# vllm-project/production-stack

Hardware: AMD Instinct MI355X
Metric: output_tokens_per_sec (higher is better)
Workload: dtype bfloat16; 1 GPU; multi-round-qa; model=llama-3-8b, users_per_gpu=320, rounds_per_conversation=10, max_model_len=8192, parallelism=dp1, prefix_caching=True, kv_cache_dtype=auto, quantization=none

## Files before the change

### csrc/attention.hip

```cpp
#include "ps_common.h"

template <int HEAD_DIM, int GQ, int BLOCK_SIZE, int NWAVES, int LOWREG,
          typename KVT, int PIPE = 0>
__global__ __launch_bounds__(NWAVES * 64, LOWREG ? 3 : 1) void paged_attn_decode_kernel(
    unsigned short* __restrict__ out,
    float* __restrict__ ws_acc,
    float* __restrict__ ws_ml,
    const unsigned short* __restrict__ q,
    const KVT* __restrict__ k_cache,
    const KVT* __restrict__ v_cache,
    const int* __restrict__ block_tables,
    const int* __restrict__ seq_lens,
    const int* __restrict__ order,
    int max_blocks, float scale, int KH, long q_stride, int window) {
  using KVTr = ps_kv_traits<KVT>;
  using kvec8 = typename KVTr::vec8;
  constexpr int D = HEAD_DIM;
  constexpr int LPG = D / 8;
  constexpr int TPW = 64 / LPG;
  static_assert(BLOCK_SIZE % TPW == 0, "block size must divide");
  static_assert(!PIPE || LOWREG, "the pipelined loop is a LOWREG variant");

  const int seq = order ? order[blockIdx.x] : blockIdx.x;
  if ((unsigned)seq >= gridDim.x) return;
  const int kvh = blockIdx.y;
  const int ctx = seq_lens[seq];
  const int wave = threadIdx.x >> 6;
  const int lane = threadIdx.x & 63;
  const int sg = lane / LPG;
  const int sl = lane % LPG;

  ps_bf16x8 qp[GQ];
  const unsigned short* qbase = q + (long)seq * q_stride + (long)kvh * GQ * D;
#pragma unroll
  for (int g = 0; g < GQ; g++)
    qp[g] = *(const ps_bf16x8*)(qbase + g * D + sl * 8);
  float qf[GQ][8];
  if constexpr (!LOWREG) {
#pragma unroll
    for (int g = 0; g < GQ; g++)
#pragma unroll
      for (int j = 0; j < 8; j++) qf[g][j] = ps_bf16_to_f32(qp[g][j]);
  }

  float m[GQ], l[GQ], acc[GQ][8];
#pragma unroll
  for (int g = 0; g < GQ; g++) {
    m[g] = PS_NEG_INF;
    l[g] = 0.f;
#pragma unroll
    for (int j = 0; j < 8; j++) acc[g][j] = 0.f;
  }

  const int nblocks = (ctx + BLOCK_SIZE - 1) / BLOCK_SIZE;
  const int win_lo = (window > 0 && ctx > window) ? ctx - window : 0;
  const int first_block = win_lo / BLOCK_SIZE;
  const int nsplit = gridDim.z;
  const int split = blockIdx.z;
  const int live_blocks = nblocks - first_block;
  const int per_split = (live_blocks + nsplit - 1) / nsplit;
  const int b_begin = first_block + split * per_split;
  const int b_end = min(nblocks, b_begin + per_split);
  const int* bt = block_tables + (long)seq * max_blocks;
  constexpr int TPB = BLOCK_SIZE / TPW;
  if constexpr (PIPE != 0) {
    int b = b_begin + wave;
    if (b < b_end) {
      const int lane_off = sg * D + sl * 8;
      long blk = __builtin_amdgcn_readfirstlane(bt[b]);
      for (; b < b_end; b += NWAVES) {
        const long blk_next = __builtin_amdgcn_readfirstlane(
            bt[b + NWAVES < b_end ? b + NWAVES : b]);
        const KVT* kb = k_cache + ((blk * KH + kvh) * BLOCK_SIZE) * D;
        const KVT* vb = v_cache + ((blk * KH + kvh) * BLOCK_SIZE) * D;
        const int valid_tokens = min(BLOCK_SIZE, ctx - b * BLOCK_SIZE);
        float sc[GQ][TPB];
        kvec8 vv[TPB];
#pragma unroll
        for (int g = 0; g < GQ; g++)
          asm volatile("" : "+v"(qp[g]));
#pragma unroll
        for (int tt = 0; tt < TPB; tt++) {
          const int tok = tt * TPW + sg;
          const bool valid =
              tok < valid_tokens && b * BLOCK_SIZE + tok >= win_lo;
          kvec8 kv = *(const kvec8*)(kb + tt * TPW * D + lane_off);
          float kf[8];
          KVTr::to_f32x8(kv, kf);
#pragma unroll
          for (int g = 0; g < GQ; g++) {
            float s = 0.f;
#pragma unroll
            for (int j = 0; j < 8; j++)
              s += ps_bf16_to_f32(qp[g][j]) * kf[j];
            s = ps_group_sum<LPG>(s) * scale;
            sc[g][tt] = valid ? s : PS_NEG_INF;
          }
        }
#pragma unroll
        for (int tt = 0; tt < TPB; tt++)
          vv[tt] = *(const kvec8*)(vb + tt * TPW * D + lane_off);
#pragma unroll
        for (int g = 0; g < GQ; g++) {
          float bmax = sc[g][0];
#pragma unroll
          for (int tt = 1; tt < TPB; tt++) bmax = fmaxf(bmax, sc[g][tt]);
          const float mnew = fmaxf(m[g], bmax);
          const float corr = __expf(m[g] - mnew);
          float p[TPB];
          float psum = 0.f;
#pragma unroll
          for (int tt = 0; tt < TPB; tt++) {
            p[tt] = sc[g][tt] > PS_NEG_INF ? __expf(sc[g][tt] - mnew) : 0.f;
            psum += p[tt];
          }
          l[g] = l[g] * corr + psum;
#pragma unroll
          for (int j = 0; j < 8; j++) acc[g][j] *= corr;
#pragma unroll
          for (int tt = 0; tt < TPB; tt++) {
            float vf[8];
            KVTr::to_f32x8(vv[tt], vf);
#pragma unroll
            for (int j = 0; j < 8; j++) acc[g][j] += p[tt] * vf[j];
          }
          m[g] = mnew;
        }
        blk = blk_next;
      }
    }
  }
  for (int b = PIPE ? b_end : b_begin + wave; b < b_end; b += NWAVES) {
    const long blk = bt[b];
    const KVT* kb = k_cache + ((blk * KH + kvh) * BLOCK_SIZE) * D;
    const KVT* vb = v_cache + ((blk * KH + kvh) * BLOCK_SIZE) * D;
    const int valid_tokens = min(BLOCK_SIZE, ctx - b * BLOCK_SIZE);
    float sc[GQ][TPB];
    kvec8 vv[TPB];
    if constexpr (LOWREG) {
#pragma unroll
      for (int g = 0; g < GQ; g++)
        asm volatile("" : "+v"(qp[g]));
    }
#pragma unroll
    for (int tt = 0; tt < TPB; tt++) {
      const int tok = tt * TPW + sg;
      const bool valid =
          tok < valid_tokens && b * BLOCK_SIZE + tok >= win_lo;
      kvec8 kv = *(const kvec8*)(kb + tok * D + sl * 8);
      if constexpr (!LOWREG)
        vv[tt] = *(const kvec8*)(vb + tok * D + sl * 8);
      float kf[8];
      KVTr::to_f32x8(kv, kf);
#pragma unroll
      for (int g = 0; g < GQ; g++) {
        float s = 0.f;
#pragma unroll
        for (int j = 0; j < 8; j++) {
          if constexpr (LOWREG)
            s += ps_bf16_to_f32(qp[g][j]) * kf[j];
          else
            s += qf[g][j] * kf[j];
        }
        s = ps_group_sum<LPG>(s) * scale;
        sc[g][tt] = valid ? s : PS_NEG_INF;
      }
    }
    if constexpr (LOWREG) {
#pragma unroll
      for (int tt = 0; tt < TPB; tt++)
        vv[tt] = *(const kvec8*)(vb + (tt * TPW + sg) * D + sl * 8);
    }
#pragma unroll
    for (int g = 0; g < GQ; g++) {
      float bmax = sc[g][0];
#pragma unroll
      for (int tt = 1; tt < TPB; tt++) bmax = fmaxf(bmax, sc[g][tt]);
      const float mnew = fmaxf(m[g], bmax);
      const float corr = __expf(m[g] - mnew);
      float p[TPB];
      float psum = 0.f;
#pragma unroll
      for (int tt = 0; tt < TPB; tt++) {
        p[tt] = sc[g][tt] > PS_NEG_INF ? __expf(sc[g][tt] - mnew) : 0.f;
        psum += p[tt];
      }
      l[g] = l[g] * corr + psum;
#pragma unroll
      for (int j = 0; j < 8; j++) acc[g][j] *= corr;
#pragma unroll
      for (int tt = 0; tt < TPB; tt++) {
        float vf[8];
        KVTr::to_f32x8(vv[tt], vf);
#pragma unroll
        for (int j = 0; j < 8; j++) acc[g][j] += p[tt] * vf[j];
      }
      m[g] = mnew;
    }
  }

#pragma unroll
  for (int off = LPG; off < 64; off <<= 1) {
#pragma unroll
    for (int g = 0; g < GQ; g++) {
      const float mo = __shfl_xor(m[g], off, 64);
      const float lo = __shfl_xor(l[g], off, 64);
      const float mnew = fmaxf(m[g], mo);
      const float c1 = __expf(m[g] - mnew);
      const float c2 = __expf(mo - mnew);
#pragma unroll
      for (int j = 0; j < 8; j++) {
        const float ao = __shfl_xor(acc[g][j], off, 64);
        acc[g][j] = acc[g][j] * c1 + ao * c2;
      }
      l[g] = l[g] * c1 + lo * c2;
      m[g] = mnew;
    }
  }

  __shared__ float sm[NWAVES][GQ];
  __shared__ float slse[NWAVES][GQ];
  __shared__ float sacc[NWAVES][GQ][D];
  if (sg == 0) {
#pragma unroll
    for (int g = 0; g < GQ; g++) {
      if (sl == 0) {
        sm[wave][g] = m[g];
        slse[wave][g] = l[g];
      }
#pragma unroll
      for (int j = 0; j < 8; j++) sacc[wave][g][sl * 8 + j] = acc[g][j];
    }
  }
  __syncthreads();
  if (wave == 0 && sg == 0) {
#pragma unroll
    for (int g = 0; g < GQ; g++) {
      float M = PS_NEG_INF, L = 0.f, A[8];
#pragma unroll
      for (int j = 0; j < 8; j++) A[j] = 0.f;
#pragma unroll
      for (int wv = 0; wv < NWAVES; wv++) {
        const float mw = sm[wv][g];
        const float mnew = fmaxf(M, mw);
        const float c1 = __expf(M - mnew);
        const float c2 = __expf(mw - mnew);
        L = L * c1 + slse[wv][g] * c2;
#pragma unroll
        for (int j = 0; j < 8; j++)
          A[j] = A[j] * c1 + sacc[wv][g][sl * 8 + j] * c2;
        M = mnew;
      }
      const long head = (long)seq * KH * GQ + (long)kvh * GQ + g;
      if (nsplit == 1) {
        const float inv = L > 0.f ? 1.f / L : 0.f;
        ps_bf16x8 ov;
#pragma unroll
        for (int j = 0; j < 8; j++) ov[j] = ps_f32_to_bf16(A[j] * inv);
        *(ps_bf16x8*)(out + head * D + sl * 8) = ov;
      } else {
        float* wa = ws_acc + (head * nsplit + split) * D + sl * 8;
#pragma unroll
        for (int j = 0; j < 8; j++) wa[j] = A[j];
        if (sl == 0) {
          float* wm = ws_ml + (head * nsplit + split) * 2;
          wm[0] = M;
          wm[1] = L;
        }
      }
    }
  }
}

#define PS_DECODE_ORDER_MAX 4096
__global__ __launch_bounds__(1024) void decode_order_kernel(
    int* __restrict__ order,
    const int* __restrict__ seq_lens,
    int S) {
  __shared__ int lens[PS_DECODE_ORDER_MAX];
  for (int i = threadIdx.x; i < S; i += blockDim.x) lens[i] = seq_lens[i];
  __syncthreads();
// ... 86 lines not shown
    const long blk = bt[b];
    const unsigned short* kb = k_cache + ((blk * KH + kvh) * BLOCK_SIZE) * D;
    const unsigned short* vb = v_cache + ((blk * KH + kvh) * BLOCK_SIZE) * D;
    const int valid_tokens = min(BLOCK_SIZE, ctx - b * BLOCK_SIZE);
#pragma unroll
    for (int tt = 0; tt < BLOCK_SIZE / TPW; tt++) {
      const int tok = tt * TPW + sg;
      const bool valid =
          tok < valid_tokens && b * BLOCK_SIZE + tok >= win_lo;
      ps_bf16x8 kv = *(const ps_bf16x8*)(kb + tok * D + sl * 8);
      ps_bf16x8 vv = *(const ps_bf16x8*)(vb + tok * D + sl * 8);
      float s = 0.f;
#pragma unroll
      for (int j = 0; j < 8; j++) s += qf[j] * ps_bf16_to_f32(kv[j]);
      s = ps_group_sum<LPG>(s);
      const float sv = valid ? s : PS_NEG_INF;
      const float mnew = fmaxf(m, sv);
      const float corr = __expf(m - mnew);
      const float p = valid ? __expf(sv - mnew) : 0.f;
      l = l * corr + p;
#pragma unroll
      for (int j = 0; j < 8; j++)
        acc[j] = acc[j] * corr + p * ps_bf16_to_f32(vv[j]);
      m = mnew;
    }
  }

#pragma unroll
  for (int off = LPG; off < 64; off <<= 1) {
    const float mo = __shfl_xor(m, off, 64);
    const float lo = __shfl_xor(l, off, 64);
    const float mnew = fmaxf(m, mo);
    const float c1 = __expf(m - mnew);
    const float c2 = __expf(mo - mnew);
#pragma unroll
    for (int j = 0; j < 8; j++) {
      const float ao = __shfl_xor(acc[j], off, 64);
      acc[j] = acc[j] * c1 + ao * c2;
    }
    l = l * c1 + lo * c2;
    m = mnew;
  }
  if (sg == 0) {
    const float inv = l > 0.f ? 1.f / l : 0.f;
    ps_bf16x8 ov;
#pragma unroll
    for (int j = 0; j < 8; j++) ov[j] = ps_f32_to_bf16(acc[j] * inv);
    *(ps_bf16x8*)(out + ((long)tokid * QH + qh) * D + sl * 8) = ov;
  }
}

template <typename KVT>
__global__ void reshape_and_cache_kernel(
    const unsigned short* __restrict__ k,
    const unsigned short* __restrict__ v,
    KVT* __restrict__ k_cache,
    KVT* __restrict__ v_cache,
    const long* __restrict__ slot_mapping,
    int KH, int HD, int BS, long total ) {
  using KVTr = ps_kv_traits<KVT>;
  using kvec8 = typename KVTr::vec8;
  const long stride = (long)gridDim.x * blockDim.x;
  const int row = KH * HD;
  for (long idx = (long)blockIdx.x * blockDim.x + threadIdx.x; idx < total;
       idx += stride) {
    const long elem = idx * 8;
    const long t = elem / row;
    const int r = (int)(elem % row);
    const int h = r / HD;
    const int d = r % HD;
    const long slot = slot_mapping[t];
    if (slot < 0) continue;
    const long blk = slot / BS;
    const int off = (int)(slot % BS);
    const long dst = ((blk * KH + h) * BS + off) * (long)HD + d;
    ps_bf16x8 kv = *(const ps_bf16x8*)(k + elem);
    ps_bf16x8 vv = *(const ps_bf16x8*)(v + elem);
    kvec8 ko, vo;
#pragma unroll
    for (int j = 0; j < 8; j++) {
      ko[j] = KVTr::from_f32(ps_bf16_to_f32(kv[j]));
      vo[j] = KVTr::from_f32(ps_bf16_to_f32(vv[j]));
    }
    *(kvec8*)(k_cache + dst) = ko;
    *(kvec8*)(v_cache + dst) = vo;
  }
}

__global__ void greedy_sample_kernel(long* __restrict__ out,
                                     const unsigned short* __restrict__ logits,
                                     int V) {
  const long r = blockIdx.x;
  const unsigned short* row = logits + r * (long)V;
  float best = PS_NEG_INF;
  int besti = 0;
  for (int i = threadIdx.x * 8; i + 8 <= V; i += blockDim.x * 8) {
    ps_bf16x8 xv = *(const ps_bf16x8*)(row + i);
#pragma unroll
    for (int j = 0; j < 8; j++) {
      const float f = ps_bf16_to_f32(xv[j]);
      if (f > best) {
        best = f;
        besti = i + j;
      }
    }
  }
  const int tail_start = (V / 8) * 8;
  for (int i = tail_start + threadIdx.x; i < V; i += blockDim.x) {
    const float f = ps_bf16_to_f32(row[i]);
    if (f > best) {
      best = f;
      besti = i;
    }
  }
#pragma unroll
  for (int off = 32; off > 0; off >>= 1) {
    const float ob = __shfl_xor(best, off, 64);
    const int oi = __shfl_xor(besti, off, 64);
    if (ob > best || (ob == best && oi < besti)) {
      best = ob;
      besti = oi;
    }
  }
  __shared__ float wbest[4];
  __shared__ int wbesti[4];
  const int wave = threadIdx.x >> 6;
  if ((threadIdx.x & 63) == 0) {
    wbest[wave] = best;
    wbesti[wave] = besti;
  }
  __syncthreads();
  if (threadIdx.x == 0) {
    for (int wv = 1; wv < (int)(blockDim.x >> 6); wv++) {
      if (wbest[wv] > wbest[0] ||
          (wbest[wv] == wbest[0] && wbesti[wv] < wbesti[0])) {
        wbest[0] = wbest[wv];
        wbesti[0] = wbesti[wv];
      }
    }
    out[r] = wbesti[0];
  }
}

extern "C" {

int ps_paged_attn_decode(void* out, void* ws_acc, void* ws_ml, const void* q,
                         const void* k_cache, const void* v_cache,
                         const void* block_tables, const void* seq_lens,
                         int num_seqs, int max_blocks, float scale, int KH,
                         int GQ, int head_dim, int block_size, int num_splits,
                         long q_stride, int variant, int kv_fp8,
                         int window, const void* order,
                         hipStream_t stream) {
  if (variant < 0 || variant > 2) return -1;
  dim3 grid(num_seqs, KH, num_splits);
  constexpr int NW = 4;
  dim3 block(NW * 64);
#define PS_DECODE_T(HD, G, BS, LR, KVT, PIPE)                                \
  paged_attn_decode_kernel<HD, G, BS, NW, LR, KVT, PIPE>                     \
      <<<grid, block, 0, stream>>>(                                          \
          (unsigned short*)out, (float*)ws_acc, (float*)ws_ml,               \
          (const unsigned short*)q, (const KVT*)k_cache,                     \
          (const KVT*)v_cache, (const int*)block_tables,                     \
          (const int*)seq_lens, (const int*)order, max_blocks, scale, KH,    \
          q_stride, window)
#define PS_DECODE_V(HD, G, BS, KVT)                                          \
  do {                                                                       \
    if (variant == 2)                                                        \
      PS_DECODE_T(HD, G, BS, 1, KVT, 1);                                     \
    else if (variant == 1)                                                   \
      PS_DECODE_T(HD, G, BS, 1, KVT, 0);                                     \
    else                                                                     \
      PS_DECODE_T(HD, G, BS, 0, KVT, 0);                                     \
  } while (0)
#define PS_DISPATCH_DECODE(HD, G, BS)                                        \
  do {                                                                       \
    if (kv_fp8)                                                              \
      PS_DECODE_V(HD, G, BS, unsigned char);                                 \
    else                                                                     \
      PS_DECODE_V(HD, G, BS, unsigned short);                                \
    if (num_splits > 1)                                                      \
      paged_attn_combine_kernel<HD>                                          \
          <<<dim3(num_seqs * KH * G), 64, 0, stream>>>(                      \
              (unsigned short*)out, (const float*)ws_acc,                    \
              (const float*)ws_ml, num_splits);                              \
  } while (0)
  if (head_dim == 128 && block_size == 16) {
    switch (GQ) {
      case 1: PS_DISPATCH_DECODE(128, 1, 16); return 0;
      case 2: PS_DISPATCH_DECODE(128, 2, 16); return 0;
      case 3: PS_DISPATCH_DECODE(128, 3, 16); return 0;
      case 4: PS_DISPATCH_DECODE(128, 4, 16); return 0;
      case 6: PS_DISPATCH_DECODE(128, 6, 16); return 0;
      case 7: PS_DISPATCH_DECODE(128, 7, 16); return 0;
      case 8: PS_DISPATCH_DECODE(128, 8, 16); return 0;
      default: return -1;
    }
  }
  if (head_dim == 64 && block_size == 16 && !kv_fp8) {
    switch (GQ) {
      case 1: PS_DISPATCH_DECODE(64, 1, 16); return 0;
      case 2: PS_DISPATCH_DECODE(64, 2, 16); return 0;
      case 4: PS_DISPATCH_DECODE(64, 4, 16); return 0;
      case 8: PS_DISPATCH_DECODE(64, 8, 16); return 0;
      default: return -1;
    }
  }
  return -1;
#undef PS_DECODE_T
#undef PS_DECODE_V
#undef PS_DISPATCH_DECODE
}

int ps_decode_order(void* order, const void* seq_lens, int S,
                    hipStream_t stream) {
  if (S < 1 || S > PS_DECODE_ORDER_MAX) return -1;
  const int threads = S <= 256 ? 256 : 1024;
  decode_order_kernel<<<1, threads, 0, stream>>>((int*)order,
                                                 (const int*)seq_lens, S);
  return 0;
}

int ps_paged_attn_prefill(void* out, const void* q, const void* k_cache,
                          const void* v_cache, const void* block_tables,
                          const void* token_seq, const void* token_pos,
                          int num_tokens, int num_q_heads, int max_blocks,
                          float scale, int KH, int GQ, int head_dim,
                          int block_size, long q_stride, int window,
                          hipStream_t stream) {
  dim3 grid(num_tokens, num_q_heads);
  dim3 block(64);
#define PS_DISPATCH_PREFILL(HD, BS)                                         \
  paged_attn_prefill_kernel<HD, BS><<<grid, block, 0, stream>>>(            \
      (unsigned short*)out, (const unsigned short*)q,                       \
      (const unsigned short*)k_cache, (const unsigned short*)v_cache,       \
      (const int*)block_tables, (const int*)token_seq,                      \
      (const int*)token_pos, max_blocks, scale, KH, GQ, q_stride, window)
  if (head_dim == 128 && block_size == 16) {
    PS_DISPATCH_PREFILL(128, 16);
    return 0;
  }
  if (head_dim == 64 && block_size == 16) {
    PS_DISPATCH_PREFILL(64, 16);
    return 0;
  }
  return -1;
#undef PS_DISPATCH_PREFILL
}

void ps_reshape_and_cache(const void* k, const void* v, void* k_cache,
                          void* v_cache, const void* slot_mapping, long T,
                          int KH, int HD, int BS, int kv_fp8,
                          hipStream_t stream) {
  const long total = T * (long)KH * HD / 8;
  const int block = 256;
  const long want = (total + block - 1) / block;
  const int grid = (int)(want < 2048 ? (want > 0 ? want : 1) : 2048);
  if (kv_fp8)
    reshape_and_cache_kernel<unsigned char><<<grid, block, 0, stream>>>(
        (const unsigned short*)k, (const unsigned short*)v,
        (unsigned char*)k_cache, (unsigned char*)v_cache,
        (const long*)slot_mapping, KH, HD, BS, total);
  else
    reshape_and_cache_kernel<unsigned short><<<grid, block, 0, stream>>>(
        (const unsigned short*)k, (const unsigned short*)v,
        (unsigned short*)k_cache, (unsigned short*)v_cache,
        (const long*)slot_mapping, KH, HD, BS, total);
}

void ps_greedy_sample(void* out, const void* logits, long R, int V,
                      hipStream_t stream) {
  greedy_sample_kernel<<<dim3((unsigned)R), 256, 0, stream>>>(
      (long*)out, (const unsigned short*)logits, V);
}

}
```

### csrc/ps_common.h

```cpp
#pragma once

#include <hip/hip_fp8.h>
#include <hip/hip_runtime.h>

#define PS_DEV __device__ __forceinline__

typedef __attribute__((ext_vector_type(8))) unsigned short ps_bf16x8;
typedef __attribute__((ext_vector_type(4))) unsigned short ps_bf16x4;
typedef __attribute__((ext_vector_type(4))) float ps_f32x4;

PS_DEV float ps_bf16_to_f32(unsigned short u) {
  union {
    float f;
    unsigned int i;
  } v;
  v.i = ((unsigned int)u) << 16;
  return v.f;
}

PS_DEV unsigned short ps_f32_to_bf16(float f) {
  union {
    float f;
    unsigned int i;
  } v;
  v.f = f;
  unsigned int x = v.i;
  if ((x & 0x7fffffffu) > 0x7f800000u) return 0x7fc0;
  unsigned int r = (x >> 16) & 1u;
  x += 0x7fffu + r;
  return (unsigned short)(x >> 16);
}

template <int WIDTH>
PS_DEV float ps_group_sum(float v) {
#pragma unroll
  for (int off = WIDTH / 2; off > 0; off >>= 1) v += __shfl_xor(v, off, WIDTH);
  return v;
}

template <int WIDTH>
PS_DEV float ps_group_max(float v) {
#pragma unroll
  for (int off = WIDTH / 2; off > 0; off >>= 1)
    v = fmaxf(v, __shfl_xor(v, off, WIDTH));
  return v;
}

#define PS_NEG_INF (-3.0e38f)

typedef __attribute__((ext_vector_type(8))) unsigned char ps_fp8x8;

PS_DEV float ps_fp8_to_f32(unsigned char u) {
  __hip_fp8_e4m3 v;
  v.__x = u;
  return (float)v;
}
PS_DEV unsigned char ps_f32_to_fp8(float f) {
  return __hip_fp8_e4m3(f).__x;
}

typedef __attribute__((ext_vector_type(2))) float ps_f32x2;

PS_DEV void ps_fp8x8_to_f32(ps_fp8x8 v, float* out) {
  union {
    ps_fp8x8 v8;
    int i2[2];
  } u;
  u.v8 = v;
#pragma unroll
  for (int w = 0; w < 2; w++) {
    ps_f32x2 lo = __builtin_amdgcn_cvt_pk_f32_fp8(u.i2[w], false);
    ps_f32x2 hi = __builtin_amdgcn_cvt_pk_f32_fp8(u.i2[w], true);
    out[w * 4 + 0] = lo.x;
    out[w * 4 + 1] = lo.y;
    out[w * 4 + 2] = hi.x;
    out[w * 4 + 3] = hi.y;
  }
}

typedef __attribute__((ext_vector_type(2))) __bf16 ps_rawbf16x2;

PS_DEV ps_bf16x8 ps_fp8x8_to_bf16x8(ps_fp8x8 v) {
  float f[8];
  ps_fp8x8_to_f32(v, f);
  union {
    ps_bf16x8 v8;
    unsigned int i4[4];
  } out;
#pragma unroll
  for (int w = 0; w < 4; w++) {
    ps_f32x2 p = {f[2 * w], f[2 * w + 1]};
    ps_rawbf16x2 b = __builtin_convertvector(p, ps_rawbf16x2);
    out.i4[w] = *(unsigned int*)&b;
  }
  return out.v8;
}

template <typename KVT>
struct ps_kv_traits;

typedef __attribute__((ext_vector_type(4))) unsigned char ps_fp8x4;

template <>
struct ps_kv_traits<unsigned short> {
  using vec8 = ps_bf16x8;
  using vec4 = ps_bf16x4;
  static PS_DEV float to_f32(unsigned short u) { return ps_bf16_to_f32(u); }
  static PS_DEV unsigned short from_f32(float f) { return ps_f32_to_bf16(f); }
  static PS_DEV unsigned short to_bf16(unsigned short u) { return u; }
  static PS_DEV void to_f32x8(ps_bf16x8 v, float* out) {
#pragma unroll
    for (int j = 0; j < 8; j++) out[j] = ps_bf16_to_f32(v[j]);
  }
  static PS_DEV ps_bf16x8 to_bf16x8(ps_bf16x8 v) { return v; }
};

template <>
struct ps_kv_traits<unsigned char> {
  using vec8 = ps_fp8x8;
  using vec4 = ps_fp8x4;
  static PS_DEV float to_f32(unsigned char u) { return ps_fp8_to_f32(u); }
  static PS_DEV unsigned char from_f32(float f) { return ps_f32_to_fp8(f); }
  static PS_DEV unsigned short to_bf16(unsigned char u) {
    return ps_f32_to_bf16(ps_fp8_to_f32(u));
  }
  static PS_DEV void to_f32x8(ps_fp8x8 v, float* out) {
    ps_fp8x8_to_f32(v, out);
  }
  static PS_DEV ps_bf16x8 to_bf16x8(ps_fp8x8 v) {
    return ps_fp8x8_to_bf16x8(v);
  }
};

static inline int ps_cdiv(int a, int b) { return (a + b - 1) / b; }
```

### production_stack_amd/engine/models/llama.py

```python

from __future__ import annotations

import math
from typing import List, Optional

import torch
import torch.nn as nn
import torch.nn.functional as F

from production_stack_amd import ops
from production_stack_amd.ops import gemm_policy
from production_stack_amd.engine.config import ModelConfig
from production_stack_amd.parallel import state as pstate


class BatchMeta:

    def __init__(
        self,
        positions: torch.Tensor,
        slot_mapping: torch.Tensor,
        num_prefill_tokens: int,
        prefill_token_seq: Optional[torch.Tensor],
        prefill_token_pos: Optional[torch.Tensor],
# ... 36 lines not shown
    head_dim: int, max_position: int, theta: float,
    rope_scaling=None,
) -> torch.Tensor:
    half = head_dim // 2
    inv = 1.0 / (
        theta ** (torch.arange(0, head_dim, 2, dtype=torch.float64) / head_dim)
    )
    if rope_scaling is not None:
        factor, low_f, high_f, orig_max = rope_scaling
        low_wl = orig_max / low_f
        high_wl = orig_max / high_f
        wavelen = 2 * math.pi / inv
        scaled = torch.where(wavelen > low_wl, inv / factor, inv)
        smooth = (orig_max / wavelen - low_f) / (high_f - low_f)
        mid = (1 - smooth) * (inv / factor) + smooth * inv
        in_band = (wavelen <= low_wl) & (wavelen >= high_wl)
        inv = torch.where(in_band, mid, scaled)
    t = torch.arange(max_position, dtype=torch.float64)
    freqs = torch.outer(t, inv)
    return torch.cat([freqs.cos(), freqs.sin()], dim=-1).float().contiguous()


class LlamaLayer(nn.Module):
    def __init__(self, cfg: ModelConfig, tp: int, layer_idx: int = 0) -> None:
        super().__init__()
        self.cfg = cfg
        self.layer_idx = layer_idx
        assert cfg.num_q_heads % tp == 0, "q heads must divide TP"
        assert cfg.num_kv_heads % tp == 0 or tp % cfg.num_kv_heads == 0
        self.q_heads = cfg.num_q_heads // tp
        self.kv_heads = max(cfg.num_kv_heads // tp, 1)
        self.head_dim = cfg.head_dim
        self.inter = cfg.intermediate_size // tp
        h = cfg.hidden_size
        qs = self.q_heads * self.head_dim
        kvs = self.kv_heads * self.head_dim
        self.qkv_proj = nn.Parameter(
            torch.empty(qs + 2 * kvs, h, dtype=torch.bfloat16)
        )
        self.o_proj = nn.Parameter(torch.empty(h, qs, dtype=torch.bfloat16))
        self.n_experts = cfg.num_experts
        self.top_k = cfg.num_experts_per_tok
        self.moe_backend = "loop"
        if self.n_experts:
            self.moe_gate = nn.Parameter(
                torch.empty(self.n_experts, h, dtype=torch.bfloat16)
            )
            self.experts_gate_up = nn.Parameter(
                torch.empty(self.n_experts, 2 * self.inter, h,
                            dtype=torch.bfloat16)
            )
            self.experts_down = nn.Parameter(
                torch.empty(self.n_experts, h, self.inter,
                            dtype=torch.bfloat16)
            )
        else:
            self.gate_up_proj = nn.Parameter(
                torch.empty(2 * self.inter, h, dtype=torch.bfloat16)
            )
            self.down_proj = nn.Parameter(
                torch.empty(h, self.inter, dtype=torch.bfloat16)
            )
        self.input_norm = nn.Parameter(torch.empty(h, dtype=torch.bfloat16))
        self.post_attn_norm = nn.Parameter(
            torch.empty(h, dtype=torch.bfloat16)
        )
        self.scale = 1.0 / math.sqrt(self.head_dim)
        self.window = cfg.sliding_window or 0
        self.qkv_bias = (
            nn.Parameter(torch.empty(qs + 2 * kvs, dtype=torch.bfloat16))
            if cfg.qkv_bias else None
        )

    def forward(
        self,
        hidden: torch.Tensor,
        residual: Optional[torch.Tensor],
        meta: BatchMeta,
        kv_cache: tuple,
        cos_sin: torch.Tensor,
    ) -> tuple:
        cfg = self.cfg
        fp8 = getattr(self, "fp8_w", None)
        fuse_q = (fp8 is not None and hidden.is_cuda
                  and meta.lora_idx is None and not meta.lora_groups
                  and ops.fp8_rowwise_supported(hidden.device))
        if fuse_q:
            if residual is None:
                residual = hidden.clone()
                xq, sx = ops.rms_norm_fp8(
                    hidden, self.input_norm, cfg.rms_norm_eps)
            else:
                xq, sx = ops.rms_norm_fp8(
                    hidden, self.input_norm, cfg.rms_norm_eps,
                    residual=residual)
            qkv = ops.fp8_linear_rowwise(xq, sx, *fp8["qkv"])
        else:
            if residual is None:
                residual = hidden
                hidden = ops.rms_norm(hidden, self.input_norm,
                                      cfg.rms_norm_eps)
            else:
                hidden, residual = ops.fused_add_rms_norm(
                    hidden, residual, self.input_norm, cfg.rms_norm_eps
                )
            if fp8 is not None:
                qkv = ops.fp8_linear(hidden, *fp8["qkv"])
            else:
                qkv = gemm_policy.linear(hidden, self.qkv_proj)
        if self.qkv_bias is not None:
            qkv = qkv + self.qkv_bias
        qs = self.q_heads * self.head_dim
        kvs = self.kv_heads * self.head_dim
        slots = getattr(self, "lora_slots", None)
        if slots is not None and meta.lora_idx is not None:
            li = self.layer_idx
            slots.apply("q", li, qkv, hidden, meta.lora_idx)
            slots.apply("k", li, qkv, hidden, meta.lora_idx)
            slots.apply("v", li, qkv, hidden, meta.lora_idx)
        elif meta.lora_groups:
            from production_stack_amd.engine.lora import apply_lora_slice

            li = self.layer_idx
            apply_lora_slice(qkv, hidden, meta.lora_groups, li, "q", 0, qs)
            apply_lora_slice(qkv, hidden, meta.lora_groups, li, "k", qs, kvs)
            apply_lora_slice(
                qkv, hidden, meta.lora_groups, li, "v", qs + kvs, kvs
            )
        T = qkv.shape[0]
        k_cache, v_cache = kv_cache
        if qkv.is_cuda:
            ops.fused_rope_cache(
                qkv, meta.positions, cos_sin, meta.slot_mapping,
                k_cache, v_cache, self.q_heads, self.head_dim,
            )
            qh = qkv.view(T, -1, self.head_dim)[:, : self.q_heads]
        else:
            q = qkv[:, :qs].contiguous()
            k = qkv[:, qs : qs + kvs].contiguous()
            v = qkv[:, qs + kvs :].contiguous()
            q, k = ops.rotary_embedding(
                meta.positions, q, k, cos_sin, self.head_dim
            )
            ops.reshape_and_cache(
                k.view(T, self.kv_heads, self.head_dim),
                v.view(T, self.kv_heads, self.head_dim),
                k_cache,
                v_cache,
                meta.slot_mapping,
            )
            qh = q.view(T, self.q_heads, self.head_dim)
        outs: List[torch.Tensor] = []
        tp = meta.num_prefill_tokens
        if tp > 0:
            if (
                qh.is_cuda
                and self.head_dim == 128
                and meta.prefill_tiles is not None
            ):
                outs.append(
                    ops.paged_attn_prefill_mfma(
                        qh[:tp],
                        k_cache,
                        v_cache,
                        meta.prefill_block_tables,
                        meta.prefill_tiles,
                        self.scale,
                        self.window,
                    )
                )
            else:
                outs.append(
                    ops.paged_attn_prefill(
                        qh[:tp] if qh.is_cuda else qh[:tp].contiguous(),
                        k_cache,
                        v_cache,
                        meta.prefill_block_tables,
                        meta.prefill_token_seq,
                        meta.prefill_token_pos,
                        self.scale,
                        self.window,
                    )
                )
        if meta.num_decode_seqs > 0:
            outs.append(
                ops.paged_attn_decode(
                    qh[tp:] if qh.is_cuda else qh[tp:].contiguous(),
                    k_cache,
                    v_cache,
                    meta.decode_block_tables,
                    meta.decode_seq_lens,
                    self.scale,
                    self.window,
                    meta.decode_order,
                )
            )
        attn = torch.cat(outs, dim=0) if len(outs) > 1 else outs[0]
        if getattr(self, "fp8_w", None) is not None:
            attn_out = ops.fp8_linear(attn.reshape(T, qs),
                                      *self.fp8_w["o"])
        else:
            attn_out = gemm_policy.linear(attn.view(T, qs), self.o_proj)
        if slots is not None and meta.lora_idx is not None:
            slots.apply("o", self.layer_idx, attn_out,
                        attn.reshape(T, qs), meta.lora_idx)
        elif meta.lora_groups:
            apply_lora_slice(
                attn_out, attn.view(T, qs), meta.lora_groups,
                self.layer_idx, "o",
            )
        attn_out = pstate.tp_all_reduce(attn_out)

        if self.n_experts:
            hidden, residual = ops.fused_add_rms_norm(
                attn_out, residual, self.post_attn_norm, cfg.rms_norm_eps
            )
            mlp_out = self._moe_forward(hidden)
            mlp_out = pstate.tp_all_reduce(mlp_out)
            return mlp_out, residual
        if fuse_q:
            xq, sx = ops.rms_norm_fp8(
                attn_out, self.post_attn_norm, cfg.rms_norm_eps,
                residual=residual)
            hidden = attn_out
            gate_up = ops.fp8_linear_rowwise(xq, sx, *fp8["gate_up"])
        else:
            hidden, residual = ops.fused_add_rms_norm(
                attn_out, residual, self.post_attn_norm, cfg.rms_norm_eps
            )
            if fp8 is not None:
                gate_up = ops.fp8_linear(hidden, *fp8["gate_up"])
            else:
                gate_up = gemm_policy.linear(hidden, self.gate_up_proj)
        if slots is not None and meta.lora_idx is not None:
            slots.apply("gate", self.layer_idx, gate_up, hidden,
                        meta.lora_idx)
            slots.apply("up", self.layer_idx, gate_up, hidden,
                        meta.lora_idx)
        elif meta.lora_groups:
            apply_lora_slice(
                gate_up, hidden, meta.lora_groups, self.layer_idx,
                "gate", 0, self.inter,
            )
            apply_lora_slice(
                gate_up, hidden, meta.lora_groups, self.layer_idx,
                "up", self.inter, self.inter,
            )
        if fuse_q:
            aq, sa = ops.silu_and_mul_fp8(gate_up)
            act = gate_up[:, : self.inter]
            mlp_out = ops.fp8_linear_rowwise(aq, sa, *fp8["down"])
        else:
            act = ops.silu_and_mul(gate_up)
            if fp8 is not None:
                mlp_out = ops.fp8_linear(act, *fp8["down"])
            else:
                mlp_out = gemm_policy.linear(act, self.down_proj)
        if slots is not None and meta.lora_idx is not None:
            slots.apply("down", self.layer_idx, mlp_out, act, meta.lora_idx)
        elif meta.lora_groups:
            apply_lora_slice(
                mlp_out, act, meta.lora_groups, self.layer_idx, "down"
            )
        mlp_out = pstate.tp_all_reduce(mlp_out)
        return mlp_out, residual

    def _moe_forward(self, x: torch.Tensor) -> torch.Tensor:
        logits = F.linear(x.float(), self.moe_gate.float())
        probs = torch.softmax(logits, dim=-1)
        weights, sel = torch.topk(probs, self.top_k, dim=-1)
        weights = weights / weights.sum(dim=-1, keepdim=True)
        if (
            self.moe_backend == "fused"
            and x.is_cuda
            and ops.fused_moe_supported(
                x.shape[0], self.top_k, self.n_experts, x.shape[1],
                self.inter,
            )
        ):
            return ops.fused_moe(
                x, self.experts_gate_up, self.experts_down, sel, weights
            )
        weights = weights.to(x.dtype)
        out = torch.zeros_like(x)
        for e in range(self.n_experts):
            mask = sel == e
            rows = mask.any(dim=-1).nonzero().flatten()
            if rows.numel() == 0:
                continue
            xe = x.index_select(0, rows)
            act = ops.silu_and_mul(
                gemm_policy.linear(xe, self.experts_gate_up[e])
            )
            ye = gemm_policy.linear(act, self.experts_down[e])
            w = (weights * mask.to(weights.dtype)).sum(-1)
            out.index_add_(
                0, rows, ye * w.index_select(0, rows).unsqueeze(-1)
            )
        return out


class LlamaForCausalLM(nn.Module):

    def __init__(
        self, cfg: ModelConfig, tp: int = 1, pp_rank: int = 0,
        pp_size: int = 1,
    ) -> None:
        super().__init__()
        self.cfg = cfg
        self.tp = tp
        self.pp_rank = pp_rank
        self.pp_size = pp_size
        per = (cfg.num_layers + pp_size - 1) // pp_size
        self.layer_start = pp_rank * per
        self.layer_end = min(cfg.num_layers, self.layer_start + per)
        self.is_first = pp_rank == 0
        self.is_last = pp_rank == pp_size - 1
        if self.is_first:
            self.embed = nn.Parameter(
                torch.empty(
                    cfg.vocab_size, cfg.hidden_size, dtype=torch.bfloat16
                )
            )
        self.layers = nn.ModuleList(
            LlamaLayer(cfg, tp, layer_idx=self.layer_start + i)
            for i in range(self.layer_end - self.layer_start)
        )
        if self.is_last:
            self.final_norm = nn.Parameter(
                torch.empty(cfg.hidden_size, dtype=torch.bfloat16)
            )
            if cfg.tie_word_embeddings and self.is_first:
                self.lm_head = self.embed
            else:
                self.lm_head = nn.Parameter(
                    torch.empty(
                        cfg.vocab_size, cfg.hidden_size, dtype=torch.bfloat16
                    )
                )
        self.register_buffer(
            "cos_sin",
            build_cos_sin_cache(cfg.head_dim, cfg.max_position,
                                cfg.rope_theta, cfg.rope_scaling),
            persistent=False,
        )

    @torch.no_grad()
    def random_init(self, seed: int = 0) -> None:
        dev = next(self.parameters()).device
        gen = torch.Generator(device=dev).manual_seed(seed)
# ... 81 lines not shown
```

### production_stack_amd/ops/__init__.py

```python

from __future__ import annotations

import os
from typing import Optional

import torch

from production_stack_amd.ops import reference

try:
    from production_stack_amd import _C
except ImportError:
    _C = None

HAVE_EXT = _C is not None


def _require_ext() -> None:
    if _C is None:
        raise RuntimeError(
            "production_stack_amd._C HIP extension is not built; run "
            "`PYTORCH_ROCM_ARCH=gfx950 python setup.py build_ext --inplace`. "
            "Refusing to fall back to eager PyTorch on GPU."
        )


def rms_norm(x: torch.Tensor, w: torch.Tensor, eps: float) -> torch.Tensor:
    if x.is_cuda:
        _require_ext()
        out = torch.empty_like(x)
        _C.rms_norm(out, x, w, eps)
        return out
    return reference.rms_norm(x, w, eps)


def fused_add_rms_norm(
    x: torch.Tensor, residual: torch.Tensor, w: torch.Tensor, eps: float
) -> tuple[torch.Tensor, torch.Tensor]:
    if x.is_cuda:
        _require_ext()
        _C.fused_add_rms_norm(x, residual, w, eps)
        return x, residual
    normed, summed = reference.fused_add_rms_norm(x, residual, w, eps)
    return normed, summed


def silu_and_mul(x: torch.Tensor) -> torch.Tensor:
    if x.is_cuda:
        _require_ext()
        d = x.shape[-1] // 2
        out = torch.empty(x.shape[:-1] + (d,), dtype=x.dtype, device=x.device)
        _C.silu_and_mul(out, x)
        return out
    return reference.silu_and_mul(x)


def rotary_embedding(
    positions: torch.Tensor,
    q: torch.Tensor,
    k: torch.Tensor,
    cos_sin: torch.Tensor,
    head_dim: int,
) -> tuple[torch.Tensor, torch.Tensor]:
    if q.is_cuda:
        _require_ext()
        _C.rotary_embedding(positions, q, k, cos_sin, head_dim)
        return q, k
    return reference.rotary_embedding(positions, q, k, cos_sin, head_dim)


def fused_rope_cache(
    qkv: torch.Tensor,
    positions: torch.Tensor,
    cos_sin: torch.Tensor,
    slot_mapping: torch.Tensor,
    k_cache: torch.Tensor,
    v_cache: torch.Tensor,
    q_heads: int,
    head_dim: int,
) -> None:
    _require_ext()
    _C.fused_rope_cache(
        qkv, positions, cos_sin, slot_mapping, k_cache, v_cache, q_heads,
        head_dim,
    )


def reshape_and_cache(
    k: torch.Tensor,
    v: torch.Tensor,
    k_cache: torch.Tensor,
    v_cache: torch.Tensor,
    slot_mapping: torch.Tensor,
) -> None:
    if k_cache.is_cuda:
        _require_ext()
        _C.reshape_and_cache(
            k.view(k.shape[0], -1), v.view(v.shape[0], -1), k_cache, v_cache,
            slot_mapping,
        )
        return
    reference.reshape_and_cache(k, v, k_cache, v_cache, slot_mapping)


DECODE_VARIANT = int(os.environ.get("PS_DECODE_VARIANT", "2"))
DECODE_ORDER = os.environ.get("PS_DECODE_ORDER", "1") != "0"


def paged_attn_decode(
    q: torch.Tensor,
    k_cache: torch.Tensor,
    v_cache: torch.Tensor,
    block_tables: torch.Tensor,
    seq_lens: torch.Tensor,
    scale: float,
    window: int = 0,
    order: Optional[torch.Tensor] = None,
) -> torch.Tensor:
    if q.is_cuda:
        _require_ext()
        out = torch.empty(q.shape, dtype=q.dtype, device=q.device)
        _C.paged_attn_decode(
            out, q, k_cache, v_cache, block_tables, seq_lens, scale, 0,
            DECODE_VARIANT, window, order
        )
        return out
    return reference.paged_attn_decode(
        q, k_cache, v_cache, block_tables, seq_lens, scale, window
    )


def decode_order(seq_lens: torch.Tensor) -> Optional[torch.Tensor]:
    if seq_lens.is_cuda:
        _require_ext()
        order = torch.empty_like(seq_lens)
        if not _C.decode_order(order, seq_lens):
            return None
        return order
    return torch.argsort(-seq_lens, stable=True).int()


def paged_attn_prefill(
    q: torch.Tensor,
    k_cache: torch.Tensor,
    v_cache: torch.Tensor,
    block_tables: torch.Tensor,
    token_seq: torch.Tensor,
    token_pos: torch.Tensor,
    scale: float,
    window: int = 0,
) -> torch.Tensor:
    if q.is_cuda:
        _require_ext()
        out = torch.empty(q.shape, dtype=q.dtype, device=q.device)
        _C.paged_attn_prefill(
            out, q, k_cache, v_cache, block_tables, token_seq, token_pos,
            scale, window
        )
        return out
    return reference.paged_attn_prefill(
        q, k_cache, v_cache, block_tables, token_seq, token_pos, scale,
        window
    )


PREFILL_VARIANT = int(os.environ.get("PS_PREFILL_VARIANT", "5"))


def prefill_tile_rows(num_q_heads: int, num_kv_heads: int) -> int:
    if PREFILL_VARIANT != 5:
        return 64
    gq = max(1, num_q_heads // max(1, num_kv_heads))
    gqw = 1
    while gqw < 4 and gq % (gqw * 2) == 0:
        gqw *= 2
    return 32 * (8 // gqw)


def paged_attn_prefill_mfma(
    q: torch.Tensor,
    k_cache: torch.Tensor,
    v_cache: torch.Tensor,
    block_tables: torch.Tensor,
    tile_info: torch.Tensor,
    scale: float,
    window: int = 0,
    variant: int = None,
) -> torch.Tensor:
    _require_ext()
    out = torch.empty(q.shape, dtype=q.dtype, device=q.device)
    v = PREFILL_VARIANT if variant is None else variant
    _C.paged_attn_prefill_mfma(
        out, q, k_cache, v_cache, block_tables, tile_info, scale, v, window
    )
    return out


def greedy_sample(logits: torch.Tensor) -> torch.Tensor:
    if logits.is_cuda:
        _require_ext()
        if logits.dtype != torch.bfloat16:
            return logits.float().argmax(dim=-1)
        out = torch.empty(
            logits.shape[0], dtype=torch.long, device=logits.device
        )
        _C.greedy_sample(out, logits)
        return out
    return reference.greedy_sample(logits)


def kv_quant(x: torch.Tensor) -> tuple:
    if x.is_cuda:
        _require_ext()
        hd = x.shape[-1]
        out = torch.empty(x.shape, dtype=torch.int8, device=x.device)
        scales = torch.empty(
            x.numel() // hd, dtype=torch.float32, device=x.device
        )
        _C.kv_quant(out, scales, x)
        return out, scales
    return reference.kv_quant(x)


def kv_dequant(
    q: torch.Tensor, scales: torch.Tensor, dtype=torch.bfloat16
) -> torch.Tensor:
    if q.is_cuda:
        _require_ext()
        out = torch.empty(q.shape, dtype=dtype, device=q.device)
        _C.kv_dequant(out, q, scales)
        return out
    return reference.kv_dequant(q, scales, dtype)


def skinny_gemm(x: torch.Tensor, w: torch.Tensor) -> torch.Tensor:
    _require_ext()
    out = torch.empty(
        (x.shape[0], w.shape[0]), dtype=torch.bfloat16, device=x.device
    )
    _C.skinny_gemm(out, x, w)
    return out


def cachegen_encode(q: torch.Tensor) -> torch.Tensor:
    if _C is not None and hasattr(_C, "cachegen_encode"):
        return _C.cachegen_encode(q.contiguous().cpu())
    return reference.cachegen_encode(q)


def cachegen_decode(blob: torch.Tensor, hd: int) -> torch.Tensor:
    if _C is not None and hasattr(_C, "cachegen_decode"):
        return _C.cachegen_decode(blob.contiguous().cpu(), hd)
    return reference.cachegen_decode(blob, hd)


def gemm8p(x: torch.Tensor, w: torch.Tensor) -> torch.Tensor:
    _require_ext()
    out = torch.empty(
        (x.shape[0], w.shape[0]), dtype=torch.bfloat16, device=x.device
    )
    _C.gemm8p(out, x, w)
    return out


def lora_bgmv(
    out: torch.Tensor,
    x: torch.Tensor,
    A: torch.Tensor,
    B: torch.Tensor,
    scale: torch.Tensor,
    idx: torch.Tensor,
    col_off: int = 0,
) -> None:
    if out.is_cuda:
        _require_ext()
        _C.lora_bgmv(out, x, A, B, scale, idx, col_off)
        return
    reference.lora_bgmv(out, x, A, B, scale, idx, col_off)


FUSED_MOE_MAX_PAIRS = 1024
FUSED_MOE_MAX_EXPERTS = 64


def fused_moe_supported(T: int, top_k: int, E: int, H: int, I: int) -> bool:
    return (
        T >= 1 and 1 <= top_k <= E <= FUSED_MOE_MAX_EXPERTS
        and T * top_k <= FUSED_MOE_MAX_PAIRS
        and H >= 64 and I >= 64 and H % 64 == 0 and I % 64 == 0
    )


def fused_moe(
    x: torch.Tensor,
    experts_gate_up: torch.Tensor,
    experts_down: torch.Tensor,
    topk_ids: torch.Tensor,
    topk_weights: torch.Tensor,
) -> torch.Tensor:
    if x.is_cuda:
        _require_ext()
        T, H = x.shape
        top_k = topk_ids.shape[1]
        E, _, I = experts_down.shape
        P = T * top_k
        dev = x.device
        out = torch.empty((T, H), dtype=torch.bfloat16, device=dev)
        offsets = torch.empty(E + 1, dtype=torch.int32, device=dev)
        sorted_pairs = torch.empty(P, dtype=torch.int32, device=dev)
        act = torch.empty((P, I), dtype=torch.bfloat16, device=dev)
        y = torch.empty((P, H), dtype=torch.float32, device=dev)
        _C.fused_moe(
            out, offsets, sorted_pairs, act, y, x, experts_gate_up,
            experts_down, topk_ids.contiguous(),
            topk_weights.float().contiguous(),
        )
        return out
    return reference.fused_moe(
        x, experts_gate_up, experts_down, topk_ids, topk_weights
    )


def fp8_linear(
    x: torch.Tensor, w_q: torch.Tensor, w_scale: torch.Tensor
) -> torch.Tensor:
    if x.is_cuda:
        sx = (x.abs().amax().clamp(min=1e-6) / 448.0).to(torch.float32)
        xq = (x / sx).to(torch.float8_e4m3fn)
        if w_scale.dim() == 1:
            return fp8_linear_rowwise(
                xq, sx.expand(x.shape[0]), w_q, w_scale)
        return torch._scaled_mm(
            xq, w_q.t(), scale_a=sx, scale_b=w_scale,
            out_dtype=torch.bfloat16,
        )
    wf = w_q.float() * (
        w_scale.float()[:, None] if w_scale.dim() == 1
        else w_scale.float()
    )
    return torch.nn.functional.linear(x.float(), wf).to(x.dtype)


def fp8_quantize_weight(w: torch.Tensor):
# ... 66 lines not shown
```

Baseline: 5807 tokens/s.

## Add K-prefetch decode attention variant with DPP row reduction and shared output buffer

Adds a decode-attention variant for bf16 KV and makes it the default. It prefetches the next block's K tile one iteration ahead in registers and uses DPP row-rotate adds for the 16-lane dot-product reduction instead of shuffles. It also reorders the PV accumulation to loop over tokens outermost and reuses the score array for probabilities. Separately, prefill and decode attention now write into one preallocated buffer, which removes the torch.cat copy in mixed batches. The extra prefetch registers may lower occupancy, and the DPP reduction depends on the lane layout.

```diff
diff --git a/csrc/attention.hip b/csrc/attention.hip
--- a/csrc/attention.hip
+++ b/csrc/attention.hip
@@ -20,6 +20,8 @@
   constexpr int TPW = 64 / LPG;
   static_assert(BLOCK_SIZE % TPW == 0, "block size must divide");
   static_assert(!PIPE || LOWREG, "the pipelined loop is a LOWREG variant");
+  static_assert(PIPE < 2 || sizeof(KVT) == 2, "PIPE 2 is built for bf16 KV");
+  constexpr bool KPRE = PIPE == 2;
 
   const int seq = order ? order[blockIdx.x] : blockIdx.x;
   if ((unsigned)seq >= gridDim.x) return;
@@ -67,15 +69,34 @@
     int b = b_begin + wave;
     if (b < b_end) {
       const int lane_off = sg * D + sl * 8;
+      const long tile = (long)BLOCK_SIZE * D;
       long blk = __builtin_amdgcn_readfirstlane(bt[b]);
+      long blk_next = 0;
+      kvec8 kc[TPB];
+      if constexpr (KPRE) {
+        blk_next = __builtin_amdgcn_readfirstlane(
+            bt[b + NWAVES < b_end ? b + NWAVES : b]);
+#pragma unroll
+        for (int tt = 0; tt < TPB; tt++)
+          kc[tt] = *(const kvec8*)(k_cache + (blk * KH + kvh) * tile +
+                                   tt * TPW * D + lane_off);
+      }
       for (; b < b_end; b += NWAVES) {
-        const long blk_next = __builtin_amdgcn_readfirstlane(
-            bt[b + NWAVES < b_end ? b + NWAVES : b]);
-        const KVT* kb = k_cache + ((blk * KH + kvh) * BLOCK_SIZE) * D;
-        const KVT* vb = v_cache + ((blk * KH + kvh) * BLOCK_SIZE) * D;
+        const int b_pre = b + (KPRE ? 2 : 1) * NWAVES;
+        const long blk_pre =
+            __builtin_amdgcn_readfirstlane(bt[b_pre < b_end ? b_pre : b]);
+        const KVT* kb = k_cache + (blk * KH + kvh) * tile;
+        const KVT* vb = v_cache + (blk * KH + kvh) * tile;
         const int valid_tokens = min(BLOCK_SIZE, ctx - b * BLOCK_SIZE);
         float sc[GQ][TPB];
         kvec8 vv[TPB];
+        kvec8 kn[TPB];
+        if constexpr (KPRE) {
+          const KVT* kbn = k_cache + (blk_next * KH + kvh) * tile;
+#pragma unroll
+          for (int tt = 0; tt < TPB; tt++)
+            kn[tt] = *(const kvec8*)(kbn + tt * TPW * D + lane_off);
+        }
 #pragma unroll
         for (int g = 0; g < GQ; g++)
           asm volatile("" : "+v"(qp[g]));
@@ -84,7 +105,11 @@
           const int tok = tt * TPW + sg;
           const bool valid =
               tok < valid_tokens && b * BLOCK_SIZE + tok >= win_lo;
-          kvec8 kv = *(const kvec8*)(kb + tt * TPW * D + lane_off);
+          kvec8 kv;
+          if constexpr (KPRE)
+            kv = kc[tt];
+          else
+            kv = *(const kvec8*)(kb + tt * TPW * D + lane_off);
           float kf[8];
           KVTr::to_f32x8(kv, kf);
 #pragma unroll
@@ -93,40 +118,81 @@
 #pragma unroll
             for (int j = 0; j < 8; j++)
               s += ps_bf16_to_f32(qp[g][j]) * kf[j];
-            s = ps_group_sum<LPG>(s) * scale;
+            if constexpr (PIPE == 2 && LPG == 16)
+              s = ps_row_sum16(s) * scale;
+            else
+              s = ps_group_sum<LPG>(s) * scale;
             sc[g][tt] = valid ? s : PS_NEG_INF;
           }
         }
 #pragma unroll
         for (int tt = 0; tt < TPB; tt++)
           vv[tt] = *(const kvec8*)(vb + tt * TPW * D + lane_off);
-#pragma unroll
-        for (int g = 0; g < GQ; g++) {
-          float bmax = sc[g][0];
-#pragma unroll
-          for (int tt = 1; tt < TPB; tt++) bmax = fmaxf(bmax, sc[g][tt]);
-          const float mnew = fmaxf(m[g], bmax);
-          const float corr = __expf(m[g] - mnew);
-          float p[TPB];
-          float psum = 0.f;
-#pragma unroll
-          for (int tt = 0; tt < TPB; tt++) {
-            p[tt] = sc[g][tt] > PS_NEG_INF ? __expf(sc[g][tt] - mnew) : 0.f;
-            psum += p[tt];
+        if constexpr (PIPE >= 2) {
+#pragma unroll
+          for (int g = 0; g < GQ; g++) {
+            float bmax = sc[g][0];
+#pragma unroll
+            for (int tt = 1; tt < TPB; tt++) bmax = fmaxf(bmax, sc[g][tt]);
+            const float mnew = fmaxf(m[g], bmax);
+            const float corr = __expf(m[g] - mnew);
+            float psum = 0.f;
+#pragma unroll
+            for (int tt = 0; tt < TPB; tt++) {
+              sc[g][tt] =
+                  sc[g][tt] > PS_NEG_INF ? __expf(sc[g][tt] - mnew) : 0.f;
+              psum += sc[g][tt];
+            }
+            l[g] = l[g] * corr + psum;
+#pragma unroll
+            for (int j = 0; j < 8; j++) acc[g][j] *= corr;
+            m[g] = mnew;
           }
-          l[g] = l[g] * corr + psum;
-#pragma unroll
-          for (int j = 0; j < 8; j++) acc[g][j] *= corr;
 #pragma unroll
           for (int tt = 0; tt < TPB; tt++) {
             float vf[8];
             KVTr::to_f32x8(vv[tt], vf);
 #pragma unroll
-            for (int j = 0; j < 8; j++) acc[g][j] += p[tt] * vf[j];
+            for (int g = 0; g < GQ; g++)
+#pragma unroll
+              for (int j = 0; j < 8; j++) acc[g][j] += sc[g][tt] * vf[j];
           }
-          m[g] = mnew;
+        } else {
+#pragma unroll
+          for (int g = 0; g < GQ; g++) {
+            float bmax = sc[g][0];
+#pragma unroll
+            for (int tt = 1; tt < TPB; tt++) bmax = fmaxf(bmax, sc[g][tt]);
+            const float mnew = fmaxf(m[g], bmax);
+            const float corr = __expf(m[g] - mnew);
+            float p[TPB];
+            float psum = 0.f;
+#pragma unroll
+            for (int tt = 0; tt < TPB; tt++) {
+              p[tt] = sc[g][tt] > PS_NEG_INF ? __expf(sc[g][tt] - mnew) : 0.f;
+              psum += p[tt];
+            }
+            l[g] = l[g] * corr + psum;
+#pragma unroll
+            for (int j = 0; j < 8; j++) acc[g][j] *= corr;
+#pragma unroll
+            for (int tt = 0; tt < TPB; tt++) {
+              float vf[8];
+              KVTr::to_f32x8(vv[tt], vf);
+#pragma unroll
+              for (int j = 0; j < 8; j++) acc[g][j] += p[tt] * vf[j];
+            }
+            m[g] = mnew;
+          }
         }
-        blk = blk_next;
+        if constexpr (KPRE) {
+#pragma unroll
+          for (int tt = 0; tt < TPB; tt++) kc[tt] = kn[tt];
+          blk = blk_next;
+          blk_next = blk_pre;
+        } else {
+          blk = blk_pre;
+        }
       }
     }
   }
@@ -519,7 +585,8 @@
                          long q_stride, int variant, int kv_fp8,
                          int window, const void* order,
                          hipStream_t stream) {
-  if (variant < 0 || variant > 2) return -1;
+  if (variant < 0 || variant > 3) return -1;
+  if (kv_fp8 && variant > 2) variant = 2;
   dim3 grid(num_seqs, KH, num_splits);
   constexpr int NW = 4;
   dim3 block(NW * 64);
@@ -544,6 +611,8 @@
   do {                                                                       \
     if (kv_fp8)                                                              \
       PS_DECODE_V(HD, G, BS, unsigned char);                                 \
+    else if (variant == 3)                                                   \
+      PS_DECODE_T(HD, G, BS, 1, unsigned short, 2);                          \
     else                                                                     \
       PS_DECODE_V(HD, G, BS, unsigned short);                                \
     if (num_splits > 1)                                                      \
diff --git a/csrc/ps_common.h b/csrc/ps_common.h
--- a/csrc/ps_common.h
+++ b/csrc/ps_common.h
@@ -35,6 +35,19 @@
 PS_DEV float ps_group_sum(float v) {
 #pragma unroll
   for (int off = WIDTH / 2; off > 0; off >>= 1) v += __shfl_xor(v, off, WIDTH);
+  return v;
+}
+
+PS_DEV float ps_row_sum16(float v) {
+#define PS_ROW_ROR_ADD(K)                                                    \
+  v += __builtin_bit_cast(                                                   \
+      float, __builtin_amdgcn_update_dpp(0, __builtin_bit_cast(int, v),      \
+                                         0x120 + (K), 0xf, 0xf, true))
+  PS_ROW_ROR_ADD(8);
+  PS_ROW_ROR_ADD(4);
+  PS_ROW_ROR_ADD(2);
+  PS_ROW_ROR_ADD(1);
+#undef PS_ROW_ROR_ADD
   return v;
 }
 
diff --git a/production_stack_amd/engine/models/llama.py b/production_stack_amd/engine/models/llama.py
--- a/production_stack_amd/engine/models/llama.py
+++ b/production_stack_amd/engine/models/llama.py
@@ -212,6 +212,18 @@
             qh = q.view(T, self.q_heads, self.head_dim)
         outs: List[torch.Tensor] = []
         tp = meta.num_prefill_tokens
+        buf = None
+        if (
+            qh.is_cuda
+            and 0 < tp < T
+            and meta.num_decode_seqs > 0
+            and self.head_dim == 128
+            and meta.prefill_tiles is not None
+        ):
+            buf = torch.empty(
+                (T, self.q_heads, self.head_dim),
+                dtype=qh.dtype, device=qh.device,
+            )
         if tp > 0:
             if (
                 qh.is_cuda
@@ -227,6 +239,7 @@
                         meta.prefill_tiles,
                         self.scale,
                         self.window,
+                        out=None if buf is None else buf[:tp],
                     )
                 )
             else:
@@ -253,9 +266,13 @@
                     self.scale,
                     self.window,
                     meta.decode_order,
-                )
-            )
-        attn = torch.cat(outs, dim=0) if len(outs) > 1 else outs[0]
+                    **({} if buf is None else {"out": buf[tp:]}),
+                )
+            )
+        if buf is not None:
+            attn = buf
+        else:
+            attn = torch.cat(outs, dim=0) if len(outs) > 1 else outs[0]
         if getattr(self, "fp8_w", None) is not None:
             attn_out = ops.fp8_linear(attn.reshape(T, qs),
                                       *self.fp8_w["o"])
diff --git a/production_stack_amd/ops/__init__.py b/production_stack_amd/ops/__init__.py
--- a/production_stack_amd/ops/__init__.py
+++ b/production_stack_amd/ops/__init__.py
@@ -103,8 +103,20 @@
     reference.reshape_and_cache(k, v, k_cache, v_cache, slot_mapping)
 
 
-DECODE_VARIANT = int(os.environ.get("PS_DECODE_VARIANT", "2"))
+DECODE_VARIANT = int(os.environ.get("PS_DECODE_VARIANT", "3"))
 DECODE_ORDER = os.environ.get("PS_DECODE_ORDER", "1") != "0"
+
+
+def _check_out(out: torch.Tensor, q: torch.Tensor) -> None:
+    if (
+        out.shape != q.shape
+        or out.dtype != q.dtype
+        or out.device != q.device
+        or not out.is_contiguous()
+    ):
+        raise ValueError(
+            "out must be contiguous with q's shape, dtype and device"
+        )
 
 
 def paged_attn_decode(
@@ -116,18 +128,27 @@
     scale: float,
     window: int = 0,
     order: Optional[torch.Tensor] = None,
-) -> torch.Tensor:
+    out: Optional[torch.Tensor] = None,
+    variant: Optional[int] = None,
+) -> torch.Tensor:
+    if out is not None:
+        _check_out(out, q)
     if q.is_cuda:
         _require_ext()
-        out = torch.empty(q.shape, dtype=q.dtype, device=q.device)
+        if out is None:
+            out = torch.empty(q.shape, dtype=q.dtype, device=q.device)
         _C.paged_attn_decode(
             out, q, k_cache, v_cache, block_tables, seq_lens, scale, 0,
-            DECODE_VARIANT, window, order
-        )
-        return out
-    return reference.paged_attn_decode(
+            DECODE_VARIANT if variant is None else variant, window, order
+        )
+        return out
+    res = reference.paged_attn_decode(
         q, k_cache, v_cache, block_tables, seq_lens, scale, window
     )
+    if out is None:
+        return res
+    out.copy_(res)
+    return out
 
 
 def decode_order(seq_lens: torch.Tensor) -> Optional[torch.Tensor]:
@@ -186,9 +207,13 @@
     scale: float,
     window: int = 0,
     variant: int = None,
-) -> torch.Tensor:
-    _require_ext()
-    out = torch.empty(q.shape, dtype=q.dtype, device=q.device)
+    out: Optional[torch.Tensor] = None,
+) -> torch.Tensor:
+    _require_ext()
+    if out is None:
+        out = torch.empty(q.shape, dtype=q.dtype, device=q.device)
+    else:
+        _check_out(out, q)
     v = PREFILL_VARIANT if variant is None else variant
     _C.paged_attn_prefill_mfma(
         out, q, k_cache, v_cache, block_tables, tile_info, scale, v, window
```

Result: faster. 5983 tokens/s, median of 6 (+3.0%).
